# TheStageAI/TheWhisper

Measured on NVIDIA H100. Metric: tokens_per_sec, higher is better.
Workload: dtype bf16

## Files before the change

thewhisper_b200/csrc/api.cu:

```cuda
#include <limits.h>
#include <stdarg.h>
#include <stdlib.h>
#include <string.h>

#include <map>
#include <string>
#include <tuple>
#include <vector>

#ifdef BW_F16
#define BW_RENAME_SUFFIX _f16
#define BW_API_NS bw_api_f16
#else
#define BW_RENAME_SUFFIX _bf16
#define BW_API_NS bw_api
#endif
#include "abi_rename.h"
#include "../../include/thewhisper_b200.h"
#include "decode.cuh"
#include "decode_mega_common.cuh"
#include "kernels.h"

namespace BW_NS {

static thread_local char g_err[1024] = "";
void set_error(const char* fmt, ...) {
  va_list ap;
  va_start(ap, fmt);
  vsnprintf(g_err, sizeof(g_err), fmt, ap);
  va_end(ap);
}
const char* get_error() { return g_err; }
int g_pdl = 0;
static int g_pdl_enabled = -1;

size_t word_timestamps_work_floats(int Ha, int Tcap, int S);
int word_timestamps_batch_device(cudaStream_t st, const float* align, int Ha, int Tcap, int S, const int* items_dev, const int* slot_map_dev,
                                 int map_pitch, int n, int maxT, int maxNF, double time_precision, float* work, float* out_dev);

namespace {

struct EncLayer {
  const float *ln1g, *ln1b, *bqkv, *bo, *ln2g, *ln2b, *b1, *b2;
  const bf16 *wqkv, *wo, *w1, *w2;
};
constexpr const char* kDecQuant[6] = {"wqkv", "wo", "xwq", "xwo", "w1", "w2"};
struct DecLayer {
  const float *ln1g, *ln1b, *bqkv, *bo, *ln2g, *ln2b, *xbq, *xbv, *xbo, *ln3g, *ln3b, *b1, *b2;
  const void *wqkv, *wo, *xwq, *xwo, *w1, *w2;
  const bf16 *xwk, *xwv;
  const float* sc[6] = {nullptr, nullptr, nullptr, nullptr, nullptr, nullptr};
};

struct GraphKey {
  int A, G, begin_index, ts_rules, align, variant, eos, pad, ts_begin, no_ts;
  bool operator<(const GraphKey& o) const {
    return std::tie(A, G, begin_index, ts_rules, align, variant, eos, pad, ts_begin, no_ts) <
           std::tie(o.A, o.G, o.begin_index, o.ts_rules, o.align, o.variant, o.eos, o.pad, o.ts_begin, o.no_ts);
  }
};

}
}

using namespace BW_NS;

struct bw_engine {
  bw_config cfg;
  std::map<std::string, const void*> tensors;
  bool finalized = false;
  int D, H, S, F, V, Vp, Tmax, Spad;
  const bf16 *conv1_w = nullptr, *conv2_w = nullptr;
  const void* embed = nullptr;
  const float* embed_scale = nullptr;
  const float** wscale_tab = nullptr;
  const float *conv1_b = nullptr, *conv2_b = nullptr, *enc_pos = nullptr, *enc_lnf_g = nullptr, *enc_lnf_b = nullptr;
  const float *dec_pos = nullptr, *dec_lnf_g = nullptr, *dec_lnf_b = nullptr;
  std::vector<EncLayer> enc;
  std::vector<DecLayer> dec;
  LogmelPlan* mel_plan = nullptr;
  std::vector<int> align_pairs;
  bf16 *mel_tm = nullptr, *h1 = nullptr, *xn = nullptr, *qkv = nullptr, *vt = nullptr, *ao = nullptr, *hbuf = nullptr, *enc_out = nullptr;
  float *x_enc = nullptr, *mel_scratch = nullptr;
  unsigned* mel_max = nullptr;
  bf16 *cross_k = nullptr, *cross_v = nullptr;
  bf16 *self_k = nullptr, *self_v = nullptr;
  int *tokens = nullptr, *finished = nullptr, *pos = nullptr, *anc = nullptr, *anc_tmp = nullptr, *head_slots = nullptr;
  unsigned *done_ctr = nullptr, *xcounters = nullptr, *sup_bits = nullptr, *bsup_bits = nullptr, *sel_ctr = nullptr;
  unsigned long long* sel_best = nullptr;
  float *dx = nullptr, *dqkv = nullptr, *dattn = nullptr, *dq = nullptr, *dh = nullptr, *logits = nullptr, *part_o = nullptr,
        *part_ml = nullptr, *align = nullptr, *lse = nullptr, *ts_work = nullptr, *ts_out = nullptr;
  int *reorder_tmp = nullptr, *cand_tokens = nullptr, *ts_items = nullptr, *ts_map = nullptr;
  float *run_scores = nullptr, *cand_scores = nullptr;
  size_t align_bytes = 0;
  int A = 0, G = 1, Q = 0;
  int steps = 0;
  bw_decode_opts opts{};
  bool use_anc = false;
  std::map<GraphKey, cudaGraphExec_t> graphs;
  cudaGraphExec_t cur_graph = nullptr;
  std::map<cudaGraphExec_t, int> graph_kernels;
  long long step_kernel_launches = 0;
  bool no_graph = false, simt = false, no_mega = false, no_fused_select = false;
  int mega_flags = MEGA_DEFAULT_FLAGS;
  bf16 *dbn = nullptr, *dba = nullptr, *dbh = nullptr;
  float* dpart = nullptr;
  int batch_min = 3;
  bool gemm2 = true;
  bool attn_vdirect = true;
  long long gemm2_min_rows = 1024;
  bool enc_graph = true;
  bool enc_pdl = false;
  std::map<int, cudaGraphExec_t> enc_graphs;
  std::map<int, int> enc_calls;
  int num_sms = 132;
  unsigned* mega_bar = nullptr;
  long long* mega_trace = nullptr;
  std::map<std::string, std::pair<void*, size_t>> buffers;
};

namespace BW_API_NS {

template <typename T>
int dalloc(bw_engine* e, const char* name, T** p, size_t count, bool zero = true) {
  const size_t bytes = count * sizeof(T);
  BW_CUDA_OK(cudaMalloc(reinterpret_cast<void**>(p), bytes ? bytes : 16));
  if (zero) BW_CUDA_OK(cudaMemset(*p, 0, bytes ? bytes : 16));
  e->buffers[name] = std::make_pair(static_cast<void*>(*p), bytes);
  return 0;
}

template <typename T>
int need(bw_engine* e, const std::string& name, const T** out) {
  auto it = e->tensors.find(name);
  BW_CHECK(it != e->tensors.end() && it->second != nullptr, "weight '%s' is not bound", name.c_str());
  *out = static_cast<const T*>(it->second);
  return 0;
}

int gemm(bw_engine* e, cudaStream_t st, const GemmA& a, const bf16* W, int B, int rows, int N, int K, const GemmEpi& epi) {
  if (e->simt) return gemm_simt(st, a, W, B, rows, N, K, epi);
  if (e->gemm2 && a.kwrap >= K && a.pitch == K && a.batch_stride == (long long)rows * K && !epi.pos && gemm_tc2_supported(B * rows, N, K) &&
      (long long)B * rows >= e->gemm2_min_rows)
    return gemm_tc2(st, a.base, W, B * rows, N, K, rows, epi, 0);
  return gemm_tc(st, a, W, B, rows, N, K, epi, 0);
}

GemmA plainA(const bf16* base, int rows, int K) {
  GemmA a;
  a.base = base;
  a.batch_stride = (long long)rows * K;
  a.pitch = K;
  a.rows_base = rows;
  a.kwrap = INT_MAX;
  return a;
}

GemmEpi plainEpi(int rows, int ld) {
  GemmEpi ep;
  ep.batch_stride = (long long)rows * ld;
  ep.row_stride = ld;
  ep.head_stride = 64;
  return ep;
}

int encode_impl(bw_engine* e, int B, cudaStream_t st) {
  const int D = e->D, S = e->S, F = e->F, H = e->H, ffn = e->cfg.ffn, nm = e->cfg.n_mels;
  {
    GemmA a;
    a.base = e->mel_tm; a.batch_stride = (long long)(F + 2) * nm; a.pitch = nm; a.rows_base = F + 2; a.kwrap = nm;
    GemmEpi ep;
    ep.bias = e->conv1_b; ep.act = 1;
    ep.out_bf16 = e->h1 + D;
    ep.batch_stride = (long long)(F + 2) * D; ep.row_stride = D;
    if (int rc = gemm(e, st, a, e->conv1_w, B, F, D, 3 * nm, ep)) return rc;
  }
  {
    GemmA a;
    a.base = e->h1; a.batch_stride = (long long)(F + 2) * D; a.pitch = 2 * D; a.rows_base = (F + 2) / 2; a.kwrap = 2 * D;
    GemmEpi ep;
    ep.bias = e->conv2_b; ep.act = 1; ep.pos = e->enc_pos;
    ep.out_f32 = e->x_enc;
    ep.batch_stride = (long long)S * D; ep.row_stride = D;
    if (int rc = gemm(e, st, a, e->conv2_w, B, S, D, 3 * D, ep)) return rc;
  }
  const float scale = 0.125f;
  (void)scale;
  for (size_t l = 0; l < e->enc.size(); ++l) {
    const EncLayer& L = e->enc[l];
    if (int rc = layernorm_bf16(st, e->x_enc, L.ln1g, L.ln1b, e->xn, B * S, D)) return rc;
    {
      GemmEpi ep = plainEpi(S, 3 * D);
      ep.bias = L.bqkv; ep.out_bf16 = e->qkv;
      if (int rc = gemm(e, st, plainA(e->xn, S, D), L.wqkv, B, S, 3 * D, D, ep)) return rc;
    }
    if (e->simt) {
      if (int rc = attn_enc_simt(st, e->qkv, e->ao, B, S, H)) return rc;
    } else {
      if (e->attn_vdirect) {
        if (int rc = attn_enc_tc(st, e->qkv, nullptr, e->ao, B, S, e->Spad, H)) return rc;
      } else {
        if (int rc = transpose_v(st, e->qkv, e->vt, B, S, e->Spad, H)) return rc;
        if (int rc = attn_enc_tc(st, e->qkv, e->vt, e->ao, B, S, e->Spad, H)) return rc;
      }
    }
    {
      GemmEpi ep = plainEpi(S, D);
      ep.bias = L.bo; ep.residual = e->x_enc; ep.out_f32 = e->x_enc;
      if (int rc = gemm(e, st, plainA(e->ao, S, D), L.wo, B, S, D, D, ep)) return rc;
    }
    if (int rc = layernorm_bf16(st, e->x_enc, L.ln2g, L.ln2b, e->xn, B * S, D)) return rc;
    {
      GemmEpi ep = plainEpi(S, ffn);
      ep.bias = L.b1; ep.act = 1; ep.out_bf16 = e->hbuf;
      if (int rc = gemm(e, st, plainA(e->xn, S, D), L.w1, B, S, ffn, D, ep)) return rc;
    }
    {
      GemmEpi ep = plainEpi(S, D);
      ep.bias = L.b2; ep.residual = e->x_enc; ep.out_f32 = e->x_enc;
      if (int rc = gemm(e, st, plainA(e->hbuf, S, ffn), L.w2, B, S, D, ffn, ep)) return rc;
    }
  }
  if (int rc = layernorm_bf16(st, e->x_enc, e->enc_lnf_g, e->enc_lnf_b, e->enc_out, B * S, D)) return rc;
  const long long per_layer = (long long)e->cfg.max_audios * H * S * 64;
  for (size_t l = 0; l < e->dec.size(); ++l) {
    const DecLayer& L = e->dec[l];
    GemmEpi ep;
    ep.batch_stride = (long long)H * S * 64; ep.row_stride = 64; ep.head_stride = (long long)S * 64;
    ep.out_bf16 = e->cross_k + l * per_layer;
    if (int rc = gemm(e, st, plainA(e->enc_out, S, D), L.xwk, B, S, D, D, ep)) return rc;
    ep.bias = L.xbv;
    ep.out_bf16 = e->cross_v + l * per_layer;
    if (int rc = gemm(e, st, plainA(e->enc_out, S, D), L.xwv, B, S, D, D, ep)) return rc;
  }
  return 0;
}

constexpr int DPART_PER_ROW = 20480;

int step_batched_impl(bw_engine* e, cudaStream_t st);
int step_batched(bw_engine* e, cudaStream_t st) {
  if (g_pdl_enabled < 0) {
    const char* ev = getenv("BW_PDL");
    g_pdl_enabled = (ev && ev[0] == '0') ? 0 : 1;
  }
  g_pdl = g_pdl_enabled;
  const int rc = step_batched_impl(e, st);
  g_pdl = 0;
  return rc;
}
int step_batched_impl(bw_engine* e, cudaStream_t st) {
  const int D = e->D, H = e->H, S = e->S, ffn = e->cfg.ffn, Tmax = e->Tmax, Q = e->Q, A = e->A, G = e->G;
  const long long self_layer = (long long)e->cfg.max_audios * e->cfg.max_beams * Tmax * D;
  const long long cross_layer = (long long)e->cfg.max_audios * H * S * 64;
  const bool w8 = e->embed_scale != nullptr;
  auto proj = [&](const bf16* in, int K, const void* W, const float* sc, int N, int* ns) {
    const DecGemmPlan pl = gemm_dec_plan(Q, N, K, e->num_sms, true, w8);
    BW_CHECK((long long)pl.ksplit * N <= DPART_PER_ROW, "batched step: %d splits x N=%d exceed the partial-sum buffer", pl.ksplit, N);
    GemmEpi ep;
    ep.out_f32 = e->dpart; ep.row_stride = N;
    *ns = pl.ksplit;
    return gemm_dec(st, in, W, sc, Q, N, K, 0, ep, pl, (long long)Q * N);
  };
  if (int rc = launch_embed(st, e->embed, e->embed_scale, e->dec_pos, e->tokens, e->pos, e->dx, Q, D, Tmax)) return rc;
  int ns = 0;
  const float* pbias = nullptr;
  for (size_t l = 0; l < e->dec.size(); ++l) {
    const DecLayer& L = e->dec[l];
    bf16* kc = e->self_k + l * self_layer;
    bf16* vc = e->self_v + l * self_layer;
    if (int rc = launch_resid_ln(st, e->dx, e->dpart, ns, (long long)Q * D, pbias, L.ln1g, L.ln1b, e->dbn, Q, D)) return rc;
    if (int rc = proj(e->dbn, D, L.wqkv, L.sc[0], 3 * D, &ns)) return rc;
    {
      SelfAttnArgs s;
      s.qkv = e->dpart; s.nsplit = ns; s.split_stride = (long long)Q * 3 * D; s.qkv_bias = L.bqkv; s.q_alpha = 0.125f;
      s.kc = kc; s.vc = vc; s.kc_w = kc; s.vc_w = vc; s.anc = e->use_anc ? e->anc : nullptr; s.out_bf16 = e->dba; s.pos = e->pos;
      s.H = H; s.D = D; s.Tmax = Tmax;
      if (int rc = launch_self_attn(st, s, Q)) return rc;
    }
    if (int rc = proj(e->dba, D, L.wo, L.sc[1], D, &ns)) return rc;
    if (int rc = launch_resid_ln(st, e->dx, e->dpart, ns, (long long)Q * D, L.bo, L.ln2g, L.ln2b, e->dbn, Q, D)) return rc;
    if (int rc = proj(e->dbn, D, L.xwq, L.sc[2], D, &ns)) return rc;
    {
      CrossAttnArgs c;
      c.q = e->dpart; c.nsplit = ns; c.split_stride = (long long)Q * D; c.q_bias = L.xbq; c.q_alpha = 0.125f;
      c.kc = e->cross_k + l * cross_layer; c.vc = e->cross_v + l * cross_layer; c.out_bf16 = e->dba;
      c.part_o = e->part_o; c.part_ml = e->part_ml; c.counters = e->xcounters;
      c.S = S; c.H = H; c.D = D; c.G = G; c.pos = e->pos;
      if (e->opts.record_alignment && e->cfg.n_align_heads > 0) {
        c.align = e->align; c.head_slots = e->head_slots + l * H; c.Ha = e->cfg.n_align_heads;
        c.Tcap = e->cfg.max_align_steps; c.step_base = e->opts.begin_index;
      }
      if (int rc = launch_cross_attn(st, c, A)) return rc;
    }
    if (int rc = proj(e->dba, D, L.xwo, L.sc[3], D, &ns)) return rc;
    if (int rc = launch_resid_ln(st, e->dx, e->dpart, ns, (long long)Q * D, L.xbo, L.ln3g, L.ln3b, e->dbn, Q, D)) return rc;
    if (int rc = proj(e->dbn, D, L.w1, L.sc[4], ffn, &ns)) return rc;
    if (int rc = launch_gelu_bias(st, e->dpart, ns, (long long)Q * ffn, L.b1, e->dbh, Q, ffn)) return rc;
    if (int rc = proj(e->dbh, ffn, L.w2, L.sc[5], D, &ns)) return rc;
    pbias = L.b2;
  }
  if (int rc = launch_resid_ln(st, e->dx, e->dpart, ns, (long long)Q * D, pbias, e->dec_lnf_g, e->dec_lnf_b, e->dbn, Q, D)) return rc;
  {
    const DecGemmPlan pl = gemm_dec_plan(Q, e->V, D, e->num_sms, false, w8);
    GemmEpi ep;
    ep.out_f32 = e->logits; ep.row_stride = e->Vp;
    if (int rc = gemm_dec(st, e->dbn, e->embed, e->embed_scale, Q, e->V, D, e->V, ep, pl, 0)) return rc;
  }
  return 0;
}

// ... 259 lines not shown
}

int bw_engine_set_alignment_heads(bw_engine* e, const int32_t* pairs, int32_t n) {
  BW_CHECK(e && (pairs || n == 0), "bw_engine_set_alignment_heads: null argument");
  BW_CHECK(n == e->cfg.n_align_heads, "alignment heads: got %d pairs, config says %d", n, e->cfg.n_align_heads);
  e->align_pairs.assign(pairs, pairs + 2 * n);
  return 0;
}

int bw_engine_finalize(bw_engine* e) {
  BW_CHECK(e && !e->finalized, "bw_engine_finalize: bad engine");
  const bw_config& c = e->cfg;
  const int D = e->D, S = e->S, F = e->F, H = e->H, V = e->V, Tmax = e->Tmax, A = c.max_audios, Qm = c.max_audios * c.max_beams;
#define NEED(T, field, name) if (int rc = need<T>(e, name, &field)) return rc;
  NEED(bf16, e->conv1_w, "enc.conv1.w") NEED(float, e->conv1_b, "enc.conv1.b")
  NEED(bf16, e->conv2_w, "enc.conv2.w") NEED(float, e->conv2_b, "enc.conv2.b")
  NEED(float, e->enc_pos, "enc.pos") NEED(float, e->enc_lnf_g, "enc.lnf.g") NEED(float, e->enc_lnf_b, "enc.lnf.b")
  NEED(void, e->embed, "dec.embed") NEED(float, e->dec_pos, "dec.pos")
  NEED(float, e->dec_lnf_g, "dec.lnf.g") NEED(float, e->dec_lnf_b, "dec.lnf.b")
  e->enc.resize(c.enc_layers);
  for (int i = 0; i < c.enc_layers; ++i) {
    const std::string p = "enc." + std::to_string(i) + ".";
    EncLayer& L = e->enc[i];
    NEED(float, L.ln1g, p + "ln1.g") NEED(float, L.ln1b, p + "ln1.b") NEED(bf16, L.wqkv, p + "wqkv") NEED(float, L.bqkv, p + "bqkv")
    NEED(bf16, L.wo, p + "wo") NEED(float, L.bo, p + "bo") NEED(float, L.ln2g, p + "ln2.g") NEED(float, L.ln2b, p + "ln2.b")
    NEED(bf16, L.w1, p + "w1") NEED(float, L.b1, p + "b1") NEED(bf16, L.w2, p + "w2") NEED(float, L.b2, p + "b2")
  }
  e->dec.resize(c.dec_layers);
  for (int i = 0; i < c.dec_layers; ++i) {
    const std::string p = "dec." + std::to_string(i) + ".";
    DecLayer& L = e->dec[i];
    NEED(float, L.ln1g, p + "ln1.g") NEED(float, L.ln1b, p + "ln1.b") NEED(void, L.wqkv, p + "wqkv") NEED(float, L.bqkv, p + "bqkv")
    NEED(void, L.wo, p + "wo") NEED(float, L.bo, p + "bo") NEED(float, L.ln2g, p + "ln2.g") NEED(float, L.ln2b, p + "ln2.b")
    NEED(void, L.xwq, p + "xwq") NEED(float, L.xbq, p + "xbq") NEED(bf16, L.xwk, p + "xwk") NEED(bf16, L.xwv, p + "xwv")
    NEED(float, L.xbv, p + "xbv") NEED(void, L.xwo, p + "xwo") NEED(float, L.xbo, p + "xbo")
    NEED(float, L.ln3g, p + "ln3.g") NEED(float, L.ln3b, p + "ln3.b")
    NEED(void, L.w1, p + "w1") NEED(float, L.b1, p + "b1") NEED(void, L.w2, p + "w2") NEED(float, L.b2, p + "b2")
  }
  {
    const bool w8 = e->tensors.count("dec.embed.scale") != 0;
    std::map<std::string, bool> want;
    if (w8) NEED(float, e->embed_scale, "dec.embed.scale")
    want["dec.embed.scale"] = true;
    for (int i = 0; i < c.dec_layers; ++i) {
      for (int k = 0; k < 6; ++k) {
        const std::string n = "dec." + std::to_string(i) + "." + kDecQuant[k] + ".scale";
        want[n] = true;
        if (w8) {
          BW_CHECK(e->tensors.count(n), "int8 decoder weights: scale '%s' is not bound ('dec.embed.scale' is)", n.c_str());
          NEED(float, e->dec[i].sc[k], n)
        }
      }
    }
    for (const auto& kv : e->tensors) {
      const std::string& n = kv.first;
      if (n.size() > 6 && n.compare(n.size() - 6, 6, ".scale") == 0) {
        BW_CHECK(want.count(n), "weight '%s': only the int8 decoder matrices (dec.embed, dec.<i>.{wqkv,wo,xwq,xwo,w1,w2}) have scales", n.c_str());
        BW_CHECK(w8, "scale '%s' is bound but 'dec.embed.scale' is not: int8 decoder weights need the scales of all seven kinds", n.c_str());
      }
    }
    if (w8) {
      std::vector<const float*> tab;
      for (const DecLayer& L : e->dec) tab.insert(tab.end(), L.sc, L.sc + 6);
      if (dalloc(e, "wscale_tab", &e->wscale_tab, tab.size())) return -1;
      BW_CUDA_OK(cudaMemcpy(e->wscale_tab, tab.data(), tab.size() * sizeof(const float*), cudaMemcpyHostToDevice));
    }
  }
#undef NEED
  BW_CHECK(e->mel_plan != nullptr, "mel filter bank not set (bw_engine_set_mel_filters)");
  const size_t BS = (size_t)A * S;
  if (dalloc(e, "mel_tm", &e->mel_tm, (size_t)A * (F + 2) * c.n_mels)) return -1;
  if (dalloc(e, "mel_scratch", &e->mel_scratch, (size_t)A * F * c.n_mels)) return -1;
  if (dalloc(e, "mel_max", &e->mel_max, (size_t)A)) return -1;
  if (dalloc(e, "h1", &e->h1, (size_t)A * (F + 2) * D)) return -1;
  if (dalloc(e, "x_enc", &e->x_enc, BS * D)) return -1;
  if (dalloc(e, "xn", &e->xn, BS * D)) return -1;
  if (dalloc(e, "qkv", &e->qkv, BS * 3 * D)) return -1;
  if (dalloc(e, "vt", &e->vt, (size_t)A * H * 64 * e->Spad)) return -1;
  if (dalloc(e, "ao", &e->ao, BS * D)) return -1;
  if (dalloc(e, "hbuf", &e->hbuf, BS * c.ffn)) return -1;
  if (dalloc(e, "enc_out", &e->enc_out, BS * D)) return -1;
  if (dalloc(e, "cross_k", &e->cross_k, (size_t)c.dec_layers * A * H * S * 64, false)) return -1;
  if (dalloc(e, "cross_v", &e->cross_v, (size_t)c.dec_layers * A * H * S * 64, false)) return -1;
  if (dalloc(e, "self_k", &e->self_k, (size_t)c.dec_layers * Qm * Tmax * D, false)) return -1;
  if (dalloc(e, "self_v", &e->self_v, (size_t)c.dec_layers * Qm * Tmax * D, false)) return -1;
  if (dalloc(e, "tokens", &e->tokens, (size_t)Qm * Tmax)) return -1;
  if (dalloc(e, "tokens_tmp", &e->reorder_tmp, (size_t)Qm * Tmax + 2 * Qm)) return -1;
  if (dalloc(e, "finished", &e->finished, (size_t)Qm)) return -1;
  if (dalloc(e, "pos", &e->pos, 1)) return -1;
  if (dalloc(e, "anc", &e->anc, (size_t)Qm * Tmax)) return -1;
  if (dalloc(e, "anc_tmp", &e->anc_tmp, (size_t)Qm * Tmax)) return -1;
  if (dalloc(e, "done_ctr", &e->done_ctr, 1)) return -1;
  if (dalloc(e, "mega_bar", &e->mega_bar, 1024)) return -1;
  {
    const char* tr = getenv("BW_MEGA_TRACE");
    if (tr && tr[0] == '1' && dalloc(e, "mega_trace", &e->mega_trace, (size_t)e->num_sms * MEGA_TRACE_N * 6)) return -1;
  }
  if (dalloc(e, "xcounters", &e->xcounters, (size_t)A * H)) return -1;
  if (dalloc(e, "sel_ctr", &e->sel_ctr, 1)) return -1;
  if (dalloc(e, "sel_best", &e->sel_best, (size_t)Qm)) return -1;
  if (dalloc(e, "sup_bits", &e->sup_bits, (size_t)(V + 31) / 32)) return -1;
  if (dalloc(e, "bsup_bits", &e->bsup_bits, (size_t)(V + 31) / 32)) return -1;
  if (dalloc(e, "dx", &e->dx, (size_t)Qm * D)) return -1;
  if (dalloc(e, "dqkv", &e->dqkv, (size_t)Qm * 3 * D)) return -1;
  if (dalloc(e, "dattn", &e->dattn, (size_t)Qm * D)) return -1;
  if (dalloc(e, "dq", &e->dq, (size_t)Qm * D)) return -1;
  if (dalloc(e, "dh", &e->dh, (size_t)Qm * c.ffn)) return -1;
  if (dalloc(e, "logits", &e->logits, (size_t)Qm * e->Vp)) return -1;
  {
    const size_t qpad = ((size_t)Qm + 127) / 128 * 128;
    if (dalloc(e, "dbn", &e->dbn, qpad * D)) return -1;
    if (dalloc(e, "dba", &e->dba, qpad * D)) return -1;
    if (dalloc(e, "dbh", &e->dbh, qpad * c.ffn)) return -1;
    if (dalloc(e, "dpart", &e->dpart, (size_t)Qm * DPART_PER_ROW)) return -1;
  }
  if (dalloc(e, "lse", &e->lse, (size_t)Qm)) return -1;
  if (dalloc(e, "run_scores", &e->run_scores, (size_t)Qm)) return -1;
  if (dalloc(e, "cand_scores", &e->cand_scores, (size_t)Qm * 16)) return -1;
  if (dalloc(e, "cand_tokens", &e->cand_tokens, (size_t)Qm * 16)) return -1;
  if (dalloc(e, "part_o", &e->part_o, (size_t)A * H * XSPLIT * c.max_beams * 64)) return -1;
  if (dalloc(e, "part_ml", &e->part_ml, (size_t)A * H * XSPLIT * c.max_beams * 2)) return -1;
  if (dalloc(e, "head_slots", &e->head_slots, (size_t)c.dec_layers * H)) return -1;
  {
    std::vector<int> hs((size_t)c.dec_layers * H, -1);
    for (int i = 0; i < c.n_align_heads && 2 * i + 1 < (int)e->align_pairs.size(); ++i) {
      const int l = e->align_pairs[2 * i], h = e->align_pairs[2 * i + 1];
      BW_CHECK(l >= 0 && l < c.dec_layers && h >= 0 && h < H, "alignment head (%d,%d) out of range", l, h);
      hs[(size_t)l * H + h] = i;
    }
    BW_CUDA_OK(cudaMemcpy(e->head_slots, hs.data(), hs.size() * sizeof(int), cudaMemcpyHostToDevice));
  }
  if (c.n_align_heads > 0) {
    BW_CHECK((int)e->align_pairs.size() == 2 * c.n_align_heads, "alignment heads not set");
    if (dalloc(e, "align", &e->align, (size_t)Qm * c.n_align_heads * c.max_align_steps * S)) return -1;
    if (dalloc(e, "ts_map", &e->ts_map, (size_t)A * c.max_align_steps)) return -1;
    if (dalloc(e, "ts_work", &e->ts_work, (size_t)A * word_timestamps_work_floats(c.n_align_heads, c.max_align_steps, S), false)) return -1;
    if (dalloc(e, "ts_out", &e->ts_out, (size_t)A * (c.max_align_steps + 8))) return -1;
    if (dalloc(e, "ts_items", &e->ts_items, (size_t)A * 3)) return -1;
  }
  e->finalized = true;
  return 0;
}

int bw_engine_buffer(bw_engine* e, const char* name, void** p, size_t* bytes) {
  BW_CHECK(e && name && p, "bw_engine_buffer: null argument");
  auto it = e->buffers.find(name);
  BW_CHECK(it != e->buffers.end(), "bw_engine_buffer: unknown buffer '%s'", name);
  *p = it->second.first;
  if (bytes) *bytes = it->second.second;
  return 0;
}

int bw_logmel(bw_engine* e, const float* pcm, int32_t B, int32_t n_samples, float* mel_f32_out, void* stream) {
  BW_CHECK(e && e->finalized && pcm, "bw_logmel: bad arguments");
  BW_CHECK(B >= 1 && B <= e->cfg.max_audios, "bw_logmel: B=%d outside 1..%d", B, e->cfg.max_audios);
  BW_CHECK(n_samples == e->F * 160, "bw_logmel: n_samples=%d, expected %d for this chunk length", n_samples, e->F * 160);
  return logmel(static_cast<cudaStream_t>(stream), e->mel_plan, pcm, B, n_samples, e->F, e->mel_tm, mel_f32_out, e->mel_scratch, e->mel_max);
}

int bw_set_mel(bw_engine* e, const float* mel, int32_t B, void* stream) {
  BW_CHECK(e && e->finalized && mel, "bw_set_mel: bad arguments");
  BW_CHECK(B >= 1 && B <= e->cfg.max_audios, "bw_set_mel: B=%d outside 1..%d", B, e->cfg.max_audios);
  dim3 grid((e->F + 31) / 32, (e->cfg.n_mels + 31) / 32, B);
  mel_to_tm_kernel<<<grid, 256, 0, static_cast<cudaStream_t>(stream)>>>(mel, e->mel_tm, e->cfg.n_mels, e->F);
  BW_CUDA_OK(cudaGetLastError());
  return 0;
// ... 341 lines not shown
```

thewhisper_b200/csrc/gemm_tc.cu:

```cuda
#include <limits.h>

#include "kernels.h"

namespace BW_NS {

namespace {

constexpr int BM = 128;
constexpr int BK = 64;
constexpr int A_STAGE_BYTES = BM * BK * 2;
constexpr int THREADS = 288;
constexpr int CONSUMER_WARPS = 8;

template <int BN>
struct Cfg {
  static constexpr int STAGES = (BN == 256) ? 4 : (BN == 128) ? 6 : 8;
  static constexpr int B_STAGE_BYTES = BN * BK * 2;
  static constexpr int SMEM_BYTES = STAGES * (A_STAGE_BYTES + B_STAGE_BYTES) + 1024  + 256 ;
};

enum { EPI_GENERIC = 0, EPI_GELU = 1 , EPI_RESID = 2 , EPI_PLAIN = 3  };

struct GemmParams {
  int B, rows, N, K;
  int rows_per_item = INT_MAX;
  int fast_gelu = 0;
  int kwrap;
  int tiles_m;
  int ksplit;
  int kper;
  long long split_stride;
  GemmEpi epi;
};

__device__ __forceinline__ void tma_load_3d(void* smem_dst, const CUtensorMap* m, uint64_t* bar, int c0, int c1, int c2) {
  asm volatile(
      "cp.async.bulk.tensor.3d.shared::cluster.global.mbarrier::complete_tx::bytes [%0], [%1, {%3, %4, %5}], [%2];" ::"r"(
          smem_u32(smem_dst)),
      "l"(reinterpret_cast<uint64_t>(m)), "r"(smem_u32(bar)), "r"(c0), "r"(c1), "r"(c2)
      : "memory");
}

__device__ __forceinline__ float gelu_as(float x) {
  const float ax = fabsf(x);
  float t;
  asm("rcp.approx.ftz.f32 %0, %1;" : "=f"(t) : "f"(fmaf(0.3275911f * 0.70710678f, ax, 1.0f)));
  float q = 0.5f * 1.061405429f;
  q = fmaf(q, t, 0.5f * -1.453152027f);
  q = fmaf(q, t, 0.5f * 1.421413741f);
  q = fmaf(q, t, 0.5f * -0.284496736f);
  q = fmaf(q, t, 0.5f * 0.254829592f);
  q = (q * t) * ex2_approx((x * -0.72134752f) * x);
  return fmaf(-ax, q, fmaxf(x, 0.f));
}

template <int BN, int MODE>
__global__ void __launch_bounds__(THREADS, 1)
gemm_tc_kernel(const __grid_constant__ CUtensorMap tmA, const __grid_constant__ CUtensorMap tmW, const GemmParams p) {
  using C = Cfg<BN>;
  extern __shared__ uint8_t smem_raw[];
  uint8_t* smem = reinterpret_cast<uint8_t*>((reinterpret_cast<uintptr_t>(smem_raw) + 1023) & ~uintptr_t(1023));
  uint8_t* sA = smem;
  uint8_t* sB = smem + C::STAGES * A_STAGE_BYTES;
  uint64_t* bars = reinterpret_cast<uint64_t*>(sB + C::STAGES * C::B_STAGE_BYTES);
  uint64_t* full = bars;
  uint64_t* empty = bars + C::STAGES;

  const int warp = threadIdx.x >> 5;
  const int lane = threadIdx.x & 31;
  const int b = blockIdx.y / p.tiles_m;
  const int t0 = (blockIdx.y % p.tiles_m) * BM;
  const int n0 = blockIdx.x * BN;
  const int nk_all = (p.K + BK - 1) / BK;
  const int kb0 = (int)blockIdx.z * p.kper;
  const int nk = min(nk_all, kb0 + p.kper) - kb0;

  if (threadIdx.x == 0) {
    for (int s = 0; s < C::STAGES; ++s) {
      mbar_init(&full[s], 1);
      mbar_init(&empty[s], CONSUMER_WARPS);
    }
    fence_mbar_init();
  }
  if (warp == CONSUMER_WARPS && lane == 0) {
    tma_prefetch_desc(&tmA);
    tma_prefetch_desc(&tmW);
  }
  __syncthreads();

  if (warp == CONSUMER_WARPS) {
    if (lane == 0) {
      const int npre = nk < C::STAGES ? nk : C::STAGES;
      for (int kb = 0; kb < npre; ++kb) {
        mbar_arrive_expect_tx(&full[kb], A_STAGE_BYTES + C::B_STAGE_BYTES);
        tma_load_2d(sB + kb * C::B_STAGE_BYTES, &tmW, &full[kb], (kb0 + kb) * BK, n0);
      }
      pdl_wait();
      pdl_launch();
      for (int kb = 0; kb < nk; ++kb) {
        const int s = kb % C::STAGES;
        const uint32_t ph = (kb / C::STAGES) & 1;
        const int k = (kb0 + kb) * BK;
        if (kb >= npre) {
          mbar_wait_wg(&empty[s], ph ^ 1);
          mbar_arrive_expect_tx(&full[s], A_STAGE_BYTES + C::B_STAGE_BYTES);
          tma_load_2d(sB + s * C::B_STAGE_BYTES, &tmW, &full[s], k, n0);
        }
        tma_load_3d(sA + s * A_STAGE_BYTES, &tmA, &full[s], k % p.kwrap, t0 + k / p.kwrap, b);
      }
    }
  } else {
    const int g = warp >> 2;
    float acc[BN / 2];
#pragma unroll
    for (int i = 0; i < BN / 2; ++i) acc[i] = 0.f;
    for (int kb = 0; kb < nk; ++kb) {
      const int s = kb % C::STAGES;
      mbar_wait_wg(&full[s], (kb / C::STAGES) & 1);
      wg_fence();
      wg_kblock<BN>(acc, smem_u32(sA + s * A_STAGE_BYTES + g * (A_STAGE_BYTES / 2)), smem_u32(sB + s * C::B_STAGE_BYTES));
      wg_commit();
      wg_wait<1>();
      if (kb > 0 && lane == 0) mbar_arrive(&empty[(kb - 1) % C::STAGES]);
    }
    wg_wait<0>();
    wg_pin(acc);

    pdl_wait();
    const GemmEpi& e = p.epi;
    constexpr bool GEN = MODE == EPI_GENERIC;
    const bool do_alpha = GEN && e.alpha != 1.0f;
    const bool do_act = GEN ? e.act == 1 : MODE == EPI_GELU;
    const bool fast_gelu = GEN ? p.fast_gelu != 0 : true;
    const bool has_pos = GEN && e.pos != nullptr;
    const bool has_res = GEN ? e.residual != nullptr : MODE == EPI_RESID;
    const bool f32out = GEN ? e.out_f32 != nullptr : MODE == EPI_RESID;
    const int r = g * 64 + (warp & 3) * 16 + (lane >> 2);
#pragma unroll
    for (int h = 0; h < 2; ++h) {
      const int t = t0 + r + 8 * h;
      if (t >= p.rows) continue;
      const int bi = t / p.rows_per_item, ti = t - bi * p.rows_per_item;
      const long long row_off = (long long)(b + bi) * e.batch_stride + (long long)ti * e.row_stride + (long long)blockIdx.z * p.split_stride;
#pragma unroll
      for (int j = 0; j < BN / 8; ++j) {
        const int n = n0 + 8 * j + 2 * (lane & 3);
        if (n >= p.N) break;
        float f0 = acc[4 * j + 2 * h], f1 = acc[4 * j + 2 * h + 1];
        if (e.bias) {
          const float2 bb = __ldg(reinterpret_cast<const float2*>(e.bias + n));
          f0 += bb.x; f1 += bb.y;
        }
        if (do_alpha && n < e.alpha_cols) { f0 *= e.alpha; f1 *= e.alpha; }
        if (do_act) {
          if (fast_gelu) { f0 = gelu_as(f0); f1 = gelu_as(f1); }
          else { f0 = gelu_erf(f0); f1 = gelu_erf(f1); }
        }
        if (has_pos) {
          const float2 q = *reinterpret_cast<const float2*>(e.pos + (long long)t * p.N + n);
          f0 += q.x; f1 += q.y;
        }
        const long long off = row_off + (long long)(n >> 6) * e.head_stride + (n & 63);
        if (has_res) {
          const float2 q = *reinterpret_cast<const float2*>(e.residual + off);
          f0 += q.x; f1 += q.y;
        }
        if (f32out) *reinterpret_cast<float2*>(e.out_f32 + off) = make_float2(f0, f1);
        else *reinterpret_cast<uint32_t*>(e.out_bf16 + off) = pack_bf16(f0, f1);
      }
    }
  }
}

__global__ void gemm_simt_kernel(GemmA a, const bf16* __restrict__ W, GemmParams p) {
  const int n = blockIdx.x * 16 + threadIdx.x;
  const int t = (blockIdx.y % p.tiles_m) * 16 + threadIdx.y;
  const int b = blockIdx.y / p.tiles_m;
  if (n >= p.N || t >= p.rows) return;
  const bf16* ab = a.base + (long long)b * a.batch_stride;
  const bf16* w = W + (long long)n * p.K;
  float acc = 0.f;
  const int kend = (p.epi.n_valid > 0 && n >= p.epi.n_valid) ? 0 : p.K;
  for (int k = 0; k < kend; ++k) {
    const float av = e2f(ab[(long long)(t + k / p.kwrap) * a.pitch + (k % p.kwrap)]);
    acc = fmaf(av, e2f(w[k]), acc);
  }
  const GemmEpi& e = p.epi;
  const long long off = (long long)b * e.batch_stride + (long long)t * e.row_stride + (long long)(n >> 6) * e.head_stride + (n & 63);
  if (e.bias) acc += e.bias[n];
  if (n < e.alpha_cols) acc *= e.alpha;
  if (e.act == 1) acc = gelu_erf(acc);
  if (e.pos) acc += e.pos[(long long)t * p.N + n];
  if (e.residual) acc += e.residual[off];
  if (e.out_f32) e.out_f32[off] = acc;
  else e.out_bf16[off] = f2e(acc);
}

typedef CUresult (*EncodeTiledFn)(CUtensorMap*, CUtensorMapDataType, cuuint32_t, void*, const cuuint64_t*, const cuuint64_t*,
                                  const cuuint32_t*, const cuuint32_t*, CUtensorMapInterleave, CUtensorMapSwizzle,
                                  CUtensorMapL2promotion, CUtensorMapFloatOOBfill);

EncodeTiledFn get_encode_fn() {
  static EncodeTiledFn fn = nullptr;
  if (fn) return fn;
  void* p = nullptr;
  cudaDriverEntryPointQueryResult qres;
  cudaError_t e = cudaGetDriverEntryPoint("cuTensorMapEncodeTiled", &p, cudaEnableDefault, &qres);
  if (e != cudaSuccess || qres != cudaDriverEntryPointSuccess || !p) {
    set_error("cudaGetDriverEntryPoint(cuTensorMapEncodeTiled) failed: %s", cudaGetErrorString(e));
    return nullptr;
  }
  fn = reinterpret_cast<EncodeTiledFn>(p);
  return fn;
}

int check_epi(const GemmEpi& e, int N) {
  BW_CHECK((e.out_f32 != nullptr) != (e.out_bf16 != nullptr), "gemm: exactly one of out_f32/out_bf16 must be set");
  BW_CHECK(N % 32 == 0, "gemm: N=%d must be a multiple of 32", N);
  BW_CHECK(e.row_stride % 8 == 0 && e.batch_stride % 8 == 0 && e.head_stride % 8 == 0, "gemm: output strides must be multiples of 8");
  return 0;
}

}

int device_sms() {
  static int sms = 0;
  if (sms == 0) {
    int dev = 0, n = 0;
    if (cudaGetDevice(&dev) == cudaSuccess && cudaDeviceGetAttribute(&n, cudaDevAttrMultiProcessorCount, dev) == cudaSuccess && n > 0) sms = n;
    else return 132;
  }
  return sms;
}

int make_tmap_2d_bf16(CUtensorMap* out, const void* base, uint64_t rows, uint64_t cols, uint64_t row_pitch_bytes,
                      uint32_t box_rows, uint32_t box_cols) {
  EncodeTiledFn fn = get_encode_fn();
  if (!fn) return -1;
  cuuint64_t dims[2] = {cols, rows};
  cuuint64_t strides[1] = {row_pitch_bytes};
  cuuint32_t box[2] = {box_cols, box_rows};
  cuuint32_t es[2] = {1, 1};
  CUresult r = fn(out, BW_TMAP_DTYPE, 2, const_cast<void*>(base), dims, strides, box, es,
                  CU_TENSOR_MAP_INTERLEAVE_NONE, CU_TENSOR_MAP_SWIZZLE_128B, CU_TENSOR_MAP_L2_PROMOTION_L2_128B,
                  CU_TENSOR_MAP_FLOAT_OOB_FILL_NONE);
  BW_CHECK(r == CUDA_SUCCESS, "cuTensorMapEncodeTiled(2d rows=%llu cols=%llu pitch=%llu box=%ux%u) -> %d",
           (unsigned long long)rows, (unsigned long long)cols, (unsigned long long)row_pitch_bytes, box_rows, box_cols, (int)r);
  return 0;
}

int make_tmap_2d_u8(CUtensorMap* out, const void* base, uint64_t rows, uint64_t cols, uint64_t row_pitch_bytes, uint32_t box_rows,
                    uint32_t box_cols) {
  EncodeTiledFn fn = get_encode_fn();
  if (!fn) return -1;
  cuuint64_t dims[2] = {cols, rows};
  cuuint64_t strides[1] = {row_pitch_bytes};
  cuuint32_t box[2] = {box_cols, box_rows};
  cuuint32_t es[2] = {1, 1};
  CUresult r = fn(out, CU_TENSOR_MAP_DATA_TYPE_UINT8, 2, const_cast<void*>(base), dims, strides, box, es, CU_TENSOR_MAP_INTERLEAVE_NONE,
                  CU_TENSOR_MAP_SWIZZLE_NONE, CU_TENSOR_MAP_L2_PROMOTION_L2_128B, CU_TENSOR_MAP_FLOAT_OOB_FILL_NONE);
  BW_CHECK(r == CUDA_SUCCESS, "cuTensorMapEncodeTiled(2d u8 rows=%llu cols=%llu pitch=%llu box=%ux%u) -> %d",
           (unsigned long long)rows, (unsigned long long)cols, (unsigned long long)row_pitch_bytes, box_rows, box_cols, (int)r);
  return 0;
}

static int make_tmap_3d_bf16(CUtensorMap* out, const void* base, uint64_t batch, uint64_t rows, uint64_t cols,
                             uint64_t row_pitch_bytes, uint64_t batch_pitch_bytes, uint32_t box_rows, uint32_t box_cols) {
  EncodeTiledFn fn = get_encode_fn();
  if (!fn) return -1;
  cuuint64_t dims[3] = {cols, rows, batch};
  cuuint64_t strides[2] = {row_pitch_bytes, batch_pitch_bytes};
  cuuint32_t box[3] = {box_cols, box_rows, 1};
  cuuint32_t es[3] = {1, 1, 1};
  CUresult r = fn(out, BW_TMAP_DTYPE, 3, const_cast<void*>(base), dims, strides, box, es,
                  CU_TENSOR_MAP_INTERLEAVE_NONE, CU_TENSOR_MAP_SWIZZLE_128B, CU_TENSOR_MAP_L2_PROMOTION_L2_128B,
                  CU_TENSOR_MAP_FLOAT_OOB_FILL_NONE);
  BW_CHECK(r == CUDA_SUCCESS, "cuTensorMapEncodeTiled(3d batch=%llu rows=%llu cols=%llu pitch=%llu/%llu) -> %d",
           (unsigned long long)batch, (unsigned long long)rows, (unsigned long long)cols,
           (unsigned long long)row_pitch_bytes, (unsigned long long)batch_pitch_bytes, (int)r);
  return 0;
}

template <int BN, int MODE = EPI_GENERIC>
static int launch_tc(cudaStream_t st, const CUtensorMap& tmA, const bf16* W, const GemmParams& p) {
  using C = Cfg<BN>;
  CUtensorMap tmW;
  if (int rc = make_tmap_2d_bf16(&tmW, W, p.epi.n_valid > 0 ? p.epi.n_valid : p.N, p.K, (uint64_t)p.K * 2, BN, BK)) return rc;
  static bool attr_set = false;
  if (!attr_set) {
    BW_CUDA_OK(cudaFuncSetAttribute(gemm_tc_kernel<BN, MODE>, cudaFuncAttributeMaxDynamicSharedMemorySize, C::SMEM_BYTES));
    attr_set = true;
  }
  dim3 grid((p.N + BN - 1) / BN, p.tiles_m * p.B, p.ksplit);
  BW_CUDA_OK(launch_k(gemm_tc_kernel<BN, MODE>, grid, dim3(THREADS), (size_t)C::SMEM_BYTES, st, tmA, tmW, p));
  return 0;
}

int gemm_tc(cudaStream_t st, const GemmA& a, const bf16* W, int B, int rows, int N, int K, const GemmEpi& epi, int force_bn) {
  return gemm_tc_split(st, a, W, B, rows, N, K, epi, force_bn, 1, 0);
}

int gemm_tc_ksplit(int K, int ksplit) {
  const int nk = K / BK;
  if (ksplit > nk) ksplit = nk;
  if (ksplit < 1) ksplit = 1;
  const int kper = (nk + ksplit - 1) / ksplit;
  return (nk + kper - 1) / kper;
}

int gemm_tc_split(cudaStream_t st, const GemmA& a, const bf16* W, int B, int rows, int N, int K, const GemmEpi& epi, int force_bn,
                  int ksplit, long long split_stride) {
  if (int rc = check_epi(epi, N)) return rc;
  BW_CHECK(ksplit >= 1 && (ksplit == 1 || (epi.out_f32 && !epi.bias && !epi.residual && !epi.pos && epi.act == 0 && epi.alpha == 1.0f)),
           "gemm_tc: split-K writes raw fp32 partial sums (no bias / activation / residual)");
  BW_CHECK(K % 64 == 0, "gemm_tc: K=%d must be a multiple of 64", K);
  BW_CHECK(a.pitch % 8 == 0 && a.batch_stride % 8 == 0, "gemm_tc: A pitch/batch stride must be multiples of 8 elements");
  BW_CHECK(a.kwrap >= K || a.kwrap % 64 == 0, "gemm_tc: kwrap=%d must be a multiple of 64", a.kwrap);
  GemmParams p;
  p.B = B; p.rows = rows; p.N = N; p.K = K;
  p.kwrap = a.kwrap >= K ? INT_MAX : a.kwrap;
  p.tiles_m = (rows + BM - 1) / BM;
  p.epi = epi;
  {
    const int nk = K / BK;
    p.ksplit = gemm_tc_ksplit(K, ksplit);
    p.kper = (nk + p.ksplit - 1) / p.ksplit;
    p.split_stride = split_stride;
  }
  const uint64_t inner = (uint64_t)(a.kwrap >= K ? K : a.kwrap);
  CUtensorMap tmA;
  if (int rc = make_tmap_3d_bf16(&tmA, a.base, (uint64_t)B, (uint64_t)a.rows_base, inner, (uint64_t)a.pitch * 2,
                                 (uint64_t)(B > 1 ? a.batch_stride : (long long)a.rows_base * a.pitch) * 2, BM, BK))
    return rc;
  int bn = force_bn;
  if (bn == 0) {
    const long long tiles128 = (long long)((N + 127) / 128) * p.tiles_m * B;
    bn = (N % 256 == 0 && tiles128 >= 4 * device_sms()) ? 256 : 128;
    if (N < 128) bn = 64;
  }
  switch (bn) {
    case 32: return launch_tc<32>(st, tmA, W, p);
    case 64: return launch_tc<64>(st, tmA, W, p);
    case 128: return launch_tc<128>(st, tmA, W, p);
    case 256: return launch_tc<256>(st, tmA, W, p);
  }
  BW_CHECK(false, "gemm_tc: unsupported BN=%d", bn);
}

bool gemm_tc2_supported(int M, int N, int K) { return K % BK == 0 && K >= BK && (N % 256 == 0 || N % 128 == 0) && M >= 1; }

int gemm_tc2(cudaStream_t st, const bf16* A, const bf16* W, int M, int N, int K, int rows_per_item, const GemmEpi& epi, int force_bn) {
  BW_CHECK((epi.out_f32 != nullptr) != (epi.out_bf16 != nullptr), "gemm_tc2: exactly one of out_f32/out_bf16 must be set");
  BW_CHECK(gemm_tc2_supported(M, N, K), "gemm_tc2: unsupported shape M=%d N=%d K=%d", M, N, K);
  BW_CHECK(!epi.pos, "gemm_tc2: positional-table epilogue is not supported (conv stem stays on gemm_tc)");
  BW_CHECK(epi.row_stride % 8 == 0 && epi.batch_stride % 8 == 0 && epi.head_stride % 8 == 0, "gemm_tc2: output strides must be multiples of 8");
  GemmParams p;
  p.B = 1; p.rows = M; p.N = N; p.K = K;
  p.rows_per_item = rows_per_item > 0 ? rows_per_item : INT_MAX;
  p.fast_gelu = 1;
  p.kwrap = INT_MAX;
  p.tiles_m = (M + BM - 1) / BM;
  p.ksplit = 1; p.kper = K / BK; p.split_stride = 0;
  p.epi = epi;
  CUtensorMap tmA;
  if (int rc = make_tmap_3d_bf16(&tmA, A, 1, (uint64_t)M, (uint64_t)K, (uint64_t)K * 2, (uint64_t)M * K * 2, BM, BK)) return rc;
  int force_mode = -1;
  if (force_bn >= 1000) {
    force_mode = EPI_GENERIC;
    force_bn -= 1000;
  }
  int bn = force_bn;
  if (bn == 0) {
    bn = (N % 256 == 0) ? 256 : 128;
    if (bn == 256) {
      const int sms = device_sms();
      const long long t256 = (long long)p.tiles_m * (N / 256);
      const long long waves = (t256 + sms - 1) / sms;
      if (t256 * 10 < waves * sms * 8) bn = 128;
    }
  }
  BW_CHECK(bn == 128 || bn == 256, "gemm_tc2: unsupported tile width %d", bn);
  BW_CHECK(N % bn == 0, "gemm_tc2: N=%d is not a multiple of the tile width %d", N, bn);
  int mode = EPI_GENERIC;
  if (epi.alpha == 1.0f) {
    if (epi.act == 1 && !epi.residual && epi.out_bf16) mode = EPI_GELU;
    else if (epi.act == 0 && epi.residual && epi.out_f32) mode = EPI_RESID;
    else if (epi.act == 0 && !epi.residual && epi.out_bf16) mode = EPI_PLAIN;
  }
  if (force_mode >= 0) mode = force_mode;
#define BW_TC2_CASE(BNV, MODEV) \
  if (bn == BNV && mode == MODEV) return launch_tc<BNV, MODEV>(st, tmA, W, p);
  BW_TC2_CASE(256, EPI_GENERIC) BW_TC2_CASE(256, EPI_GELU) BW_TC2_CASE(256, EPI_RESID) BW_TC2_CASE(256, EPI_PLAIN)
  BW_TC2_CASE(128, EPI_GENERIC) BW_TC2_CASE(128, EPI_GELU) BW_TC2_CASE(128, EPI_RESID) BW_TC2_CASE(128, EPI_PLAIN)
#undef BW_TC2_CASE
  BW_CHECK(false, "gemm_tc2: no kernel for bn=%d mode=%d", bn, mode);
}

int gemm_simt(cudaStream_t st, const GemmA& a, const bf16* W, int B, int rows, int N, int K, const GemmEpi& epi) {
  if (int rc = check_epi(epi, N)) return rc;
  GemmParams p;
  p.B = B; p.rows = rows; p.N = N; p.K = K;
  p.kwrap = a.kwrap >= K ? INT_MAX : a.kwrap;
  p.tiles_m = (rows + 15) / 16;
  p.ksplit = 1; p.kper = 0; p.split_stride = 0;
  p.epi = epi;
  dim3 grid((N + 15) / 16, p.tiles_m * B);
  gemm_simt_kernel<<<grid, dim3(16, 16), 0, st>>>(a, W, p);
  BW_CUDA_OK(cudaGetLastError());
  return 0;
}

}
```

thewhisper_b200/csrc/kernels.h:

```cpp
#pragma once
#include "common.cuh"

namespace BW_NS {

struct GemmA {
  const bf16* base = nullptr;
  long long batch_stride = 0;
  long long pitch = 0;
  int rows_base = 0;
  int kwrap = 0x7fffffff;
};

struct GemmEpi {
  const float* bias = nullptr;
  float alpha = 1.0f;
  int alpha_cols = 0x7fffffff;
  int act = 0;
  const float* residual = nullptr;
  const float* pos = nullptr;
  float* out_f32 = nullptr;
  bf16* out_bf16 = nullptr;
  long long batch_stride = 0;
  long long row_stride = 0;
  long long head_stride = 64;
  int n_valid = 0;
};

int gemm_tc(cudaStream_t st, const GemmA& a, const bf16* W, int B, int rows, int N, int K, const GemmEpi& epi,
            int force_bn );
int gemm_tc_split(cudaStream_t st, const GemmA& a, const bf16* W, int B, int rows, int N, int K, const GemmEpi& epi, int force_bn,
                  int ksplit, long long split_stride);
int gemm_tc_ksplit(int K, int ksplit);
bool gemm_tc2_supported(int M, int N, int K);
int gemm_tc2(cudaStream_t st, const bf16* A, const bf16* W, int M, int N, int K, int rows_per_item, const GemmEpi& epi, int force_bn);
int gemm_simt(cudaStream_t st, const GemmA& a, const bf16* W, int B, int rows, int N, int K, const GemmEpi& epi);

struct DecGemmPlan {
  int QB = 16, q_tiles = 1, stages = 2, kper = 1, ksplit = 1;
  size_t smem = 0;
};
DecGemmPlan gemm_dec_plan(int Q, int N, int K, int num_sms, bool want_split, bool w8 = false);
int gemm_dec(cudaStream_t st, const bf16* X, const void* W, const float* wscale, int Q, int N, int K, int n_valid, const GemmEpi& epi,
             const DecGemmPlan& pl, long long split_stride);
int launch_gelu_bias(cudaStream_t st, const float* part, int nsplit, long long split_stride, const float* bias, bf16* h, int Q, int N);

int attn_enc_tc(cudaStream_t st, const bf16* qkv, const bf16* vt, bf16* out, int B, int S, int Spad, int H);
int attn_enc_simt(cudaStream_t st, const bf16* qkv, bf16* out, int B, int S, int H);
int transpose_v(cudaStream_t st, const bf16* qkv, bf16* vt, int B, int S, int Spad, int H);

int layernorm_bf16(cudaStream_t st, const float* x, const float* g, const float* b, bf16* y, int rows, int D);
int layernorm_f32(cudaStream_t st, const float* x, const float* g, const float* b, float* y, int rows, int D);

struct LogmelPlan;
int logmel_plan_create_from_bank(LogmelPlan** out, const float* bank , int n_mels);
void logmel_plan_destroy(LogmelPlan* p);
int logmel(cudaStream_t st, const LogmelPlan* plan, const float* pcm, int B, int n_samples, int frames, bf16* out_tm,
           float* out_f32, float* scratch, unsigned* scratch_max);

}
```

Measured before the change: 814.2.

## Fuse per-layer cross-attention K/V projections into one grouped GEMM launch

Replaces the 2×dec_layers separate cross K/V projection GEMMs after the encoder with a single grouped tensor-core GEMM launch. Per-group weight tensor maps, biases and output pointers are precomputed into a device table at setup. The grid is laid out with M tiles on x so that blocks sharing an A tile run together. This removes many launches and their tails and improves SM fill, at the cost of tensor maps read from global memory and more kernel complexity. It only affects encoder-side work once per audio, so the effect on decode tokens/sec is likely small.

```diff
diff --git a/thewhisper_b200/csrc/api.cu b/thewhisper_b200/csrc/api.cu
--- a/thewhisper_b200/csrc/api.cu
+++ b/thewhisper_b200/csrc/api.cu
@@ -84,6 +84,7 @@
   float *x_enc = nullptr, *mel_scratch = nullptr;
   unsigned* mel_max = nullptr;
   bf16 *cross_k = nullptr, *cross_v = nullptr;
+  GemmGroup* xkv_groups = nullptr;
   bf16 *self_k = nullptr, *self_v = nullptr;
   int *tokens = nullptr, *finished = nullptr, *pos = nullptr, *anc = nullptr, *anc_tmp = nullptr, *head_slots = nullptr;
   unsigned *done_ctr = nullptr, *xcounters = nullptr, *sup_bits = nullptr, *bsup_bits = nullptr, *sel_ctr = nullptr;
@@ -138,10 +139,13 @@
   return 0;
 }
 
+bool flat_rows(const bw_engine* e, int B, int rows, int N, int K) {
+  return !e->simt && e->gemm2 && gemm_tc2_supported(B * rows, N, K) && (long long)B * rows >= e->gemm2_min_rows;
+}
+
 int gemm(bw_engine* e, cudaStream_t st, const GemmA& a, const bf16* W, int B, int rows, int N, int K, const GemmEpi& epi) {
   if (e->simt) return gemm_simt(st, a, W, B, rows, N, K, epi);
-  if (e->gemm2 && a.kwrap >= K && a.pitch == K && a.batch_stride == (long long)rows * K && !epi.pos && gemm_tc2_supported(B * rows, N, K) &&
-      (long long)B * rows >= e->gemm2_min_rows)
+  if (a.kwrap >= K && a.pitch == K && a.batch_stride == (long long)rows * K && !epi.pos && flat_rows(e, B, rows, N, K))
     return gemm_tc2(st, a.base, W, B * rows, N, K, rows, epi, 0);
   return gemm_tc(st, a, W, B, rows, N, K, epi, 0);
 }
@@ -223,10 +227,13 @@
   }
   if (int rc = layernorm_bf16(st, e->x_enc, e->enc_lnf_g, e->enc_lnf_b, e->enc_out, B * S, D)) return rc;
   const long long per_layer = (long long)e->cfg.max_audios * H * S * 64;
+  GemmEpi ep;
+  ep.batch_stride = (long long)H * S * 64; ep.row_stride = 64; ep.head_stride = (long long)S * 64;
+  if (e->xkv_groups && flat_rows(e, B, S, D, D))
+    return gemm_tc2_grouped(st, e->enc_out, B * S, D, S, e->xkv_groups, 2 * (int)e->dec.size(), D, ep);
   for (size_t l = 0; l < e->dec.size(); ++l) {
     const DecLayer& L = e->dec[l];
-    GemmEpi ep;
-    ep.batch_stride = (long long)H * S * 64; ep.row_stride = 64; ep.head_stride = (long long)S * 64;
+    ep.bias = nullptr;
     ep.out_bf16 = e->cross_k + l * per_layer;
     if (int rc = gemm(e, st, plainA(e->enc_out, S, D), L.xwk, B, S, D, D, ep)) return rc;
     ep.bias = L.xbv;
@@ -652,6 +659,17 @@
   if (dalloc(e, "enc_out", &e->enc_out, BS * D)) return -1;
   if (dalloc(e, "cross_k", &e->cross_k, (size_t)c.dec_layers * A * H * S * 64, false)) return -1;
   if (dalloc(e, "cross_v", &e->cross_v, (size_t)c.dec_layers * A * H * S * 64, false)) return -1;
+  if (D % 128 == 0) {
+    std::vector<GemmGroup> tab(2 * c.dec_layers);
+    const long long per_layer = (long long)A * H * S * 64;
+    for (int l = 0; l < c.dec_layers; ++l) {
+      const DecLayer& L = e->dec[l];
+      if (int rc = gemm_tc2_make_group(&tab[2 * l], L.xwk, D, D, nullptr, e->cross_k + l * per_layer)) return rc;
+      if (int rc = gemm_tc2_make_group(&tab[2 * l + 1], L.xwv, D, D, L.xbv, e->cross_v + l * per_layer)) return rc;
+    }
+    if (dalloc(e, "xkv_groups", &e->xkv_groups, tab.size(), false)) return -1;
+    BW_CUDA_OK(cudaMemcpy(e->xkv_groups, tab.data(), tab.size() * sizeof(GemmGroup), cudaMemcpyHostToDevice));
+  }
   if (dalloc(e, "self_k", &e->self_k, (size_t)c.dec_layers * Qm * Tmax * D, false)) return -1;
   if (dalloc(e, "self_v", &e->self_v, (size_t)c.dec_layers * Qm * Tmax * D, false)) return -1;
   if (dalloc(e, "tokens", &e->tokens, (size_t)Qm * Tmax)) return -1;
diff --git a/thewhisper_b200/csrc/gemm_tc.cu b/thewhisper_b200/csrc/gemm_tc.cu
--- a/thewhisper_b200/csrc/gemm_tc.cu
+++ b/thewhisper_b200/csrc/gemm_tc.cu
@@ -31,6 +31,8 @@
   int kper;
   long long split_stride;
   GemmEpi epi;
+  const GemmGroup* groups = nullptr;
+  int ngroups = 1;
 };
 
 __device__ __forceinline__ void tma_load_3d(void* smem_dst, const CUtensorMap* m, uint64_t* bar, int c0, int c1, int c2) {
@@ -68,9 +70,13 @@
 
   const int warp = threadIdx.x >> 5;
   const int lane = threadIdx.x & 31;
-  const int b = blockIdx.y / p.tiles_m;
-  const int t0 = (blockIdx.y % p.tiles_m) * BM;
-  const int n0 = blockIdx.x * BN;
+  const int bx = p.groups ? blockIdx.y : blockIdx.x, by = p.groups ? blockIdx.x : blockIdx.y;
+  const int b = by / p.tiles_m;
+  const int t0 = (by % p.tiles_m) * BM;
+  const int tn = (p.N + BN - 1) / BN;
+  const GemmGroup* grp = p.groups ? p.groups + bx / tn : nullptr;
+  const CUtensorMap* tw = grp ? &grp->tmW : &tmW;
+  const int n0 = (bx % tn) * BN;
   const int nk_all = (p.K + BK - 1) / BK;
   const int kb0 = (int)blockIdx.z * p.kper;
   const int nk = min(nk_all, kb0 + p.kper) - kb0;
@@ -84,7 +90,7 @@
   }
   if (warp == CONSUMER_WARPS && lane == 0) {
     tma_prefetch_desc(&tmA);
-    tma_prefetch_desc(&tmW);
+    tma_prefetch_desc(tw);
   }
   __syncthreads();
 
@@ -93,7 +99,7 @@
       const int npre = nk < C::STAGES ? nk : C::STAGES;
       for (int kb = 0; kb < npre; ++kb) {
         mbar_arrive_expect_tx(&full[kb], A_STAGE_BYTES + C::B_STAGE_BYTES);
-        tma_load_2d(sB + kb * C::B_STAGE_BYTES, &tmW, &full[kb], (kb0 + kb) * BK, n0);
+        tma_load_2d(sB + kb * C::B_STAGE_BYTES, tw, &full[kb], (kb0 + kb) * BK, n0);
       }
       pdl_wait();
       pdl_launch();
@@ -104,7 +110,7 @@
         if (kb >= npre) {
           mbar_wait_wg(&empty[s], ph ^ 1);
           mbar_arrive_expect_tx(&full[s], A_STAGE_BYTES + C::B_STAGE_BYTES);
-          tma_load_2d(sB + s * C::B_STAGE_BYTES, &tmW, &full[s], k, n0);
+          tma_load_2d(sB + s * C::B_STAGE_BYTES, tw, &full[s], k, n0);
         }
         tma_load_3d(sA + s * A_STAGE_BYTES, &tmA, &full[s], k % p.kwrap, t0 + k / p.kwrap, b);
       }
@@ -128,6 +134,8 @@
 
     pdl_wait();
     const GemmEpi& e = p.epi;
+    const float* bias = grp ? grp->bias : e.bias;
+    bf16* out16 = grp ? grp->out : e.out_bf16;
     constexpr bool GEN = MODE == EPI_GENERIC;
     const bool do_alpha = GEN && e.alpha != 1.0f;
     const bool do_act = GEN ? e.act == 1 : MODE == EPI_GELU;
@@ -147,8 +155,8 @@
         const int n = n0 + 8 * j + 2 * (lane & 3);
         if (n >= p.N) break;
         float f0 = acc[4 * j + 2 * h], f1 = acc[4 * j + 2 * h + 1];
-        if (e.bias) {
-          const float2 bb = __ldg(reinterpret_cast<const float2*>(e.bias + n));
+        if (bias) {
+          const float2 bb = __ldg(reinterpret_cast<const float2*>(bias + n));
           f0 += bb.x; f1 += bb.y;
         }
         if (do_alpha && n < e.alpha_cols) { f0 *= e.alpha; f1 *= e.alpha; }
@@ -166,7 +174,7 @@
           f0 += q.x; f1 += q.y;
         }
         if (f32out) *reinterpret_cast<float2*>(e.out_f32 + off) = make_float2(f0, f1);
-        else *reinterpret_cast<uint32_t*>(e.out_bf16 + off) = pack_bf16(f0, f1);
+        else *reinterpret_cast<uint32_t*>(out16 + off) = pack_bf16(f0, f1);
       }
     }
   }
@@ -284,14 +292,16 @@
 template <int BN, int MODE = EPI_GENERIC>
 static int launch_tc(cudaStream_t st, const CUtensorMap& tmA, const bf16* W, const GemmParams& p) {
   using C = Cfg<BN>;
-  CUtensorMap tmW;
-  if (int rc = make_tmap_2d_bf16(&tmW, W, p.epi.n_valid > 0 ? p.epi.n_valid : p.N, p.K, (uint64_t)p.K * 2, BN, BK)) return rc;
+  CUtensorMap tmW{};
+  if (!p.groups)
+    if (int rc = make_tmap_2d_bf16(&tmW, W, p.epi.n_valid > 0 ? p.epi.n_valid : p.N, p.K, (uint64_t)p.K * 2, BN, BK)) return rc;
   static bool attr_set = false;
   if (!attr_set) {
     BW_CUDA_OK(cudaFuncSetAttribute(gemm_tc_kernel<BN, MODE>, cudaFuncAttributeMaxDynamicSharedMemorySize, C::SMEM_BYTES));
     attr_set = true;
   }
   dim3 grid((p.N + BN - 1) / BN, p.tiles_m * p.B, p.ksplit);
+  if (p.groups) grid = dim3(p.tiles_m, grid.x * p.ngroups, 1);
   BW_CUDA_OK(launch_k(gemm_tc_kernel<BN, MODE>, grid, dim3(THREADS), (size_t)C::SMEM_BYTES, st, tmA, tmW, p));
   return 0;
 }
@@ -396,6 +406,37 @@
   BW_CHECK(false, "gemm_tc2: no kernel for bn=%d mode=%d", bn, mode);
 }
 
+int gemm_tc2_group_width(int group_n) { return group_n % 256 == 0 ? 256 : 128; }
+
+int gemm_tc2_make_group(GemmGroup* g, const bf16* W, int group_n, int K, const float* bias, bf16* out) {
+  BW_CHECK(group_n % 128 == 0 && K % BK == 0, "gemm_tc2_make_group: unsupported shape %d x %d", group_n, K);
+  g->bias = bias;
+  g->out = out;
+  return make_tmap_2d_bf16(&g->tmW, W, group_n, K, (uint64_t)K * 2, gemm_tc2_group_width(group_n), BK);
+}
+
+int gemm_tc2_grouped(cudaStream_t st, const bf16* A, int M, int K, int rows_per_item, const GemmGroup* groups, int ngroups, int group_n,
+                     const GemmEpi& epi) {
+  BW_CHECK(groups && ngroups >= 1 && gemm_tc2_supported(M, group_n, K), "gemm_tc2_grouped: unsupported launch M=%d N=%d x %d K=%d", M,
+           group_n, ngroups, K);
+  BW_CHECK(!epi.pos && !epi.residual && epi.act == 0 && epi.alpha == 1.0f, "gemm_tc2_grouped: bias -> 16 bit epilogue only");
+  BW_CHECK(epi.row_stride % 8 == 0 && epi.batch_stride % 8 == 0 && epi.head_stride % 8 == 0, "gemm_tc2_grouped: output strides must be multiples of 8");
+  GemmParams p;
+  p.B = 1; p.rows = M; p.N = group_n; p.K = K;
+  p.rows_per_item = rows_per_item > 0 ? rows_per_item : INT_MAX;
+  p.fast_gelu = 1;
+  p.kwrap = INT_MAX;
+  p.tiles_m = (M + BM - 1) / BM;
+  p.ksplit = 1; p.kper = K / BK; p.split_stride = 0;
+  p.epi = epi;
+  p.groups = groups;
+  p.ngroups = ngroups;
+  CUtensorMap tmA;
+  if (int rc = make_tmap_3d_bf16(&tmA, A, 1, (uint64_t)M, (uint64_t)K, (uint64_t)K * 2, (uint64_t)M * K * 2, BM, BK)) return rc;
+  if (gemm_tc2_group_width(group_n) == 256) return launch_tc<256, EPI_PLAIN>(st, tmA, nullptr, p);
+  return launch_tc<128, EPI_PLAIN>(st, tmA, nullptr, p);
+}
+
 int gemm_simt(cudaStream_t st, const GemmA& a, const bf16* W, int B, int rows, int N, int K, const GemmEpi& epi) {
   if (int rc = check_epi(epi, N)) return rc;
   GemmParams p;
diff --git a/thewhisper_b200/csrc/kernels.h b/thewhisper_b200/csrc/kernels.h
--- a/thewhisper_b200/csrc/kernels.h
+++ b/thewhisper_b200/csrc/kernels.h
@@ -33,6 +33,15 @@
 int gemm_tc_ksplit(int K, int ksplit);
 bool gemm_tc2_supported(int M, int N, int K);
 int gemm_tc2(cudaStream_t st, const bf16* A, const bf16* W, int M, int N, int K, int rows_per_item, const GemmEpi& epi, int force_bn);
+struct GemmGroup {
+  CUtensorMap tmW;
+  const float* bias;
+  bf16* out;
+};
+int gemm_tc2_group_width(int group_n);
+int gemm_tc2_make_group(GemmGroup* g, const bf16* W, int group_n, int K, const float* bias, bf16* out);
+int gemm_tc2_grouped(cudaStream_t st, const bf16* A, int M, int K, int rows_per_item, const GemmGroup* groups, int ngroups, int group_n,
+                     const GemmEpi& epi);
 int gemm_simt(cudaStream_t st, const GemmA& a, const bf16* W, int B, int rows, int N, int K, const GemmEpi& epi);
 
 struct DecGemmPlan {
```

New measurement: 811.7 (median of 6 runs). No clear change (-0.3%).
